# sdroh1027/DiffusionVID

Hardware: AMD Instinct MI355X
Metric: frames/sec (1000x600) DiffusionVID-R101 x1 (higher is better)
Workload: dtype f16

## Files before the change

diffusionvid_amd/csrc/bneck.hip:

```cpp
#include <stdlib.h>

#include "../../include/dvid_hip.h"
#include "common.h"
#include "igemm_epilogue.h"
#include "kernels.h"
#include "options.h"

namespace {

__device__ __attribute__((aligned(16))) unsigned int g_zero16_bn[4] = {0u, 0u, 0u, 0u};

typedef unsigned int uint4v __attribute__((ext_vector_type(4)));

template <int N>
__device__ __forceinline__ void bn_wait_vmcnt() {
    asm volatile("s_waitcnt vmcnt(%0)" ::"n"(N) : "memory");
}
__device__ __forceinline__ void bn_glds16(const void* gsrc, char* lds_wave_base) {
    __builtin_amdgcn_global_load_lds((const __attribute__((address_space(1))) void*)gsrc,
                                     (__attribute__((address_space(3))) void*)lds_wave_base, 16, 0, 0);
}
__device__ __forceinline__ float bn_mix_add_lo(unsigned int h2, float x) {
    float d;
    asm("v_fma_mix_f32 %0, %1, 1.0, %2 op_sel_hi:[1,0,0]" : "=v"(d) : "v"(h2), "v"(x));
    return d;
}
__device__ __forceinline__ float bn_mix_add_hi(unsigned int h2, float x) {
    float d;
    asm("v_fma_mix_f32 %0, %1, 1.0, %2 op_sel:[1,0,0] op_sel_hi:[1,0,0]" : "=v"(d) : "v"(h2), "v"(x));
    return d;
}

constexpr int TH = 8, TW = 32;
constexpr int HH = TH + 2, HW = 34;
constexpr int PXB = 128;
constexpr int A_PIECES = 48;
constexpr int kHalo = 0;
constexpr int kW2 = A_PIECES * 1024;
constexpr int kW3 = kW2 + 9 * 8192;
constexpr int kBias = kW3 + 32768;
constexpr int kBytes = 160 * 1024;

struct BneckParams {
    const half_t* t1;
    const half_t* w2;
    const float* b2;
    const half_t* w3;
    const float* b3;
    const half_t* res;
    const half_t* ws;
    const float* bs;
    const half_t* w1n;
    const float* b1n;
    half_t* out;
    half_t* t1n;
    int H, W, nrows, tiles_x, ntiles;
};

__device__ __forceinline__ void bn_swap(const float16v& acc, unsigned int (&u)[16]) {
#pragma unroll
    for (int r = 0; r < 16; ++r) {
        const float f = acc[r];
        u[r] = __float_as_uint(f);
    }
#pragma unroll
    for (int g = 0; g < 2; ++g)
#pragma unroll
        for (int r = 0; r < 4; ++r) {
            const auto sw = __builtin_amdgcn_permlane32_swap(u[8 * g + r], u[8 * g + 4 + r], false, false);
            u[8 * g + r] = sw[0];
            u[8 * g + 4 + r] = sw[1];
        }
}

template <bool SC, int TN>
__global__ __launch_bounds__(512) void bneck64_tail_kernel(BneckParams p) {
    constexpr bool TAIL = TN > 0;
    constexpr int NT1 = TN > 0 ? TN / 32 : 1;
    constexpr int kW1 = TN == 128 ? kW2 : kHalo;
    static_assert(TN == 0 || TN == 64 || (TN == 128 && !SC), "next conv1: 64 channels, or 128 without a shortcut in the same launch");
    extern __shared__ __attribute__((aligned(16))) char smem[];
    const int tid = threadIdx.x, lane = tid & 63;
    const int wave = __builtin_amdgcn_readfirstlane(tid >> 6);
    const int hi = lane >> 5, frow = lane & 31;
    const int lid = igemm_xcd_remap((int)blockIdx.x, p.ntiles);
    const int tx = lid % p.tiles_x, ty = lid / p.tiles_x;
    const int r0 = ty * TH, x0 = tx * TW;
    const char* zero = reinterpret_cast<const char*>(g_zero16_bn);

    if (wave < 4) {
        const float* src = wave == 0 ? p.b2 : wave == 1 ? p.b3 : wave == 2 ? (TAIL ? p.b1n : nullptr) : (SC ? p.bs : nullptr);
        const int n16 = (wave & 1) ? 64 : (wave == 2 ? TN / 4 : 16);
        bn_glds16(src && lane < n16 ? reinterpret_cast<const char*>(src + lane * 4) : zero, smem + kBias + wave * 1024);
    }
    const int prow = lane >> 3, pslot = lane & 7;
#pragma unroll
    for (int i = 0; i < A_PIECES / 8; ++i) {
        const int q = wave + 8 * i;
        const int pidx = 8 * q + prow;
        const int hy = pidx / HW, hx = pidx - hy * HW;
        const int gr = r0 - 1 + hy, gx = x0 - 1 + hx;
        const bool ok = pidx < HH * HW && (unsigned)gr < (unsigned)p.nrows && (unsigned)gx < (unsigned)p.W;
        const int lch = pslot ^ ((hx >> 1) & 7);
        bn_glds16(ok ? reinterpret_cast<const char*>(p.t1 + ((long)gr * p.W + gx) * 64 + lch * 8) : zero, smem + kHalo + q * 1024);
    }
    const int wrow = 8 * wave + prow;
    const int wlch = pslot ^ ((wrow >> 1) & 7);
    const char* const w2src = reinterpret_cast<const char*>(p.w2 + (long)wrow * 576 + wlch * 8);
#pragma unroll
    for (int tap = 0; tap < 3; ++tap) bn_glds16(w2src + tap * 128, smem + kW2 + tap * 8192 + wave * 1024);
    asm volatile("" ::: "memory");
#pragma unroll
    for (int tap = 3; tap < 9; ++tap) bn_glds16(w2src + tap * 128, smem + kW2 + tap * 8192 + wave * 1024);
#pragma unroll
    for (int i = 0; i < 4; ++i) {
        const int row = 64 * i + wrow;
        bn_glds16(reinterpret_cast<const char*>(p.w3 + (long)row * 64 + wlch * 8), smem + kW3 + i * 8192 + wave * 1024);
    }
    asm volatile("" ::: "memory");

    const int gr = r0 + wave, gx = x0 + frow;
    const bool valid = gr < p.nrows && gx < p.W;
    const long pix = (long)(gr < p.nrows ? gr : p.nrows - 1) * p.W + (gx < p.W ? gx : p.W - 1);
    constexpr int NRES = SC ? 4 : 16;
    half8 resv[NRES];
    int a_off[3][4];
#pragma unroll
    for (int dx = 0; dx < 3; ++dx)
#pragma unroll
        for (int ks = 0; ks < 4; ++ks) {
            const int hx = dx + frow;
            a_off[dx][ks] = hx * PXB + (((2 * ks + hi) ^ ((hx >> 1) & 7)) << 4);
        }
    int b_off[4];
#pragma unroll
    for (int ks = 0; ks < 4; ++ks) b_off[ks] = frow * PXB + (((2 * ks + hi) ^ ((frow >> 1) & 7)) << 4);
    const int yimg = (r0 + wave) % p.H;
    const bool up_ok = yimg > 0, down_ok = yimg < p.H - 1;

    float16v acc2[2];
#pragma unroll
    for (int j = 0; j < 2; ++j)
#pragma unroll
        for (int r = 0; r < 16; ++r) acc2[j][r] = 0.f;

    auto conv2_tap = [&](int tap) {
        const int dy = tap / 3, dx = tap % 3;
        if ((dy == 0 && !up_ok) || (dy == 2 && !down_ok)) return;
        const char* bst = smem + kW2 + tap * 8192;
        const char* hrow = smem + kHalo + (wave + dy) * (HW * PXB);
        half8 fw[2][4], fp[4];
#pragma unroll
        for (int ks = 0; ks < 4; ++ks) {
            fp[ks] = *reinterpret_cast<const half8*>(hrow + a_off[dx][ks]);
#pragma unroll
            for (int j = 0; j < 2; ++j) fw[j][ks] = *reinterpret_cast<const half8*>(bst + j * 4096 + b_off[ks]);
        }
#pragma unroll
        for (int ks = 0; ks < 4; ++ks)
#pragma unroll
            for (int j = 0; j < 2; ++j) acc2[j] = __builtin_amdgcn_mfma_f32_32x32x16_f16(fw[j][ks], fp[ks], acc2[j], 0, 0, 0);
    };

    bn_wait_vmcnt<10>();
    asm volatile("s_waitcnt lgkmcnt(0)" ::: "memory");
    __builtin_amdgcn_s_barrier();
#pragma unroll
    for (int tap = 0; tap < 3; ++tap) conv2_tap(tap);
    bn_wait_vmcnt<0>();
    __builtin_amdgcn_s_barrier();
    asm volatile("" ::: "memory");
    if (SC) {
#pragma unroll
        for (int ks = 0; ks < 4; ++ks) resv[ks] = *reinterpret_cast<const half8*>(p.res + pix * 64 + 16 * ks + 8 * hi);
    } else {
#pragma unroll
        for (int k = 0; k < 16; ++k) resv[k] = *reinterpret_cast<const half8*>(p.res + pix * 256 + 16 * k + 8 * hi);
    }
    asm volatile("" ::: "memory");
#pragma unroll
    for (int tap = 3; tap < 9; ++tap) conv2_tap(tap);
    asm volatile("s_waitcnt lgkmcnt(0)" ::: "memory");
    __builtin_amdgcn_s_barrier();
    asm volatile("" ::: "memory");

    if (TAIL) {
#pragma unroll
        for (int c = 0; c < 4; ++c)
#pragma unroll
            for (int i = 0; i < TN / 64; ++i)
                bn_glds16(reinterpret_cast<const char*>(p.w1n + (long)(64 * i + wrow) * 256 + c * 64 + wlch * 8),
                          smem + kW1 + c * (TN * 128) + (8 * i + wave) * 1024);
    }
    if (SC) {
#pragma unroll
        for (int i = 0; i < 4; ++i) {
            const int row = 64 * i + wrow;
            bn_glds16(reinterpret_cast<const char*>(p.ws + (long)row * 64 + wlch * 8), smem + kW2 + i * 8192 + wave * 1024);
        }
    }
    asm volatile("" ::: "memory");

    const float* const bl = reinterpret_cast<const float*>(smem + kBias);
    half8 t2f[4];
#pragma unroll
    for (int j = 0; j < 2; ++j) {
        unsigned int u[16];
        bn_swap(acc2[j], u);
#pragma unroll
        for (int g = 0; g < 2; ++g) {
            const float4v blo = *reinterpret_cast<const float4v*>(bl + 32 * j + 16 * g + 8 * hi);
            const float4v bhi = *reinterpret_cast<const float4v*>(bl + 32 * j + 16 * g + 8 * hi + 4);
            float4v lo, hv;
#pragma unroll
            for (int e = 0; e < 4; ++e) {
                lo[e] = __uint_as_float(u[8 * g + e]) + blo[e];
                hv[e] = __uint_as_float(u[8 * g + 4 + e]) + bhi[e];
            }
            const half4 hlo = __builtin_convertvector(lo, half4), hhi = __builtin_convertvector(hv, half4);
            half8 o = __builtin_shufflevector(hlo, hhi, 0, 1, 2, 3, 4, 5, 6, 7);
            t2f[2 * j + g] = __builtin_elementwise_max(o, half8{0, 0, 0, 0, 0, 0, 0, 0});
        }
    }
    if (TAIL || SC) {
        bn_wait_vmcnt<0>();
        __builtin_amdgcn_s_barrier();
        asm volatile("" ::: "memory");
    }

    half8 outf[16];
    half_t* const orow = p.out + ((long)gr * p.W + gx) * 256 + 8 * hi;
#pragma unroll
    for (int jj = 0; jj < 8; ++jj) {
        half8 fw3[4];
#pragma unroll
        for (int ks = 0; ks < 4; ++ks) fw3[ks] = *reinterpret_cast<const half8*>(smem + kW3 + jj * 4096 + b_off[ks]);
        float16v acc3;
#pragma unroll
        for (int r = 0; r < 16; ++r) acc3[r] = 0.f;
#pragma unroll
        for (int ks = 0; ks < 4; ++ks) acc3 = __builtin_amdgcn_mfma_f32_32x32x16_f16(fw3[ks], t2f[ks], acc3, 0, 0, 0);
        unsigned int us[16];
        if (SC) {
            half8 fws[4];
#pragma unroll
            for (int ks = 0; ks < 4; ++ks) fws[ks] = *reinterpret_cast<const half8*>(smem + kW2 + jj * 4096 + b_off[ks]);
            float16v accs;
#pragma unroll
            for (int r = 0; r < 16; ++r) accs[r] = 0.f;
#pragma unroll
            for (int ks = 0; ks < 4; ++ks) accs = __builtin_amdgcn_mfma_f32_32x32x16_f16(fws[ks], resv[ks], accs, 0, 0, 0);
            bn_swap(accs, us);
        }
        unsigned int u[16];
        bn_swap(acc3, u);
#pragma unroll
        for (int g = 0; g < 2; ++g) {
            const int c0 = 32 * jj + 16 * g + 8 * hi;
            const float4v blo = *reinterpret_cast<const float4v*>(bl + 256 + c0);
            const float4v bhi = *reinterpret_cast<const float4v*>(bl + 256 + c0 + 4);
            float4v lo, hv;
#pragma unroll
            for (int e = 0; e < 4; ++e) {
                lo[e] = __uint_as_float(u[8 * g + e]) + blo[e];
                hv[e] = __uint_as_float(u[8 * g + 4 + e]) + bhi[e];
            }
            uint4v rr;
            if (SC) {
                const float4v slo = *reinterpret_cast<const float4v*>(bl + 768 + c0);
                const float4v shi = *reinterpret_cast<const float4v*>(bl + 768 + c0 + 4);
                float4v a, b;
#pragma unroll
                for (int e = 0; e < 4; ++e) {
                    a[e] = __uint_as_float(us[8 * g + e]) + slo[e];
                    b[e] = __uint_as_float(us[8 * g + 4 + e]) + shi[e];
                }
                const half4 ha = __builtin_convertvector(a, half4), hb = __builtin_convertvector(b, half4);
                rr = __builtin_bit_cast(uint4v, __builtin_shufflevector(ha, hb, 0, 1, 2, 3, 4, 5, 6, 7));
            } else {
                rr = __builtin_bit_cast(uint4v, resv[2 * jj + g]);
            }
            lo[0] = bn_mix_add_lo(rr[0], lo[0]);
            lo[1] = bn_mix_add_hi(rr[0], lo[1]);
            lo[2] = bn_mix_add_lo(rr[1], lo[2]);
            lo[3] = bn_mix_add_hi(rr[1], lo[3]);
            hv[0] = bn_mix_add_lo(rr[2], hv[0]);
            hv[1] = bn_mix_add_hi(rr[2], hv[1]);
            hv[2] = bn_mix_add_lo(rr[3], hv[2]);
            hv[3] = bn_mix_add_hi(rr[3], hv[3]);
            const half4 hlo = __builtin_convertvector(lo, half4), hhi = __builtin_convertvector(hv, half4);
            half8 o = __builtin_shufflevector(hlo, hhi, 0, 1, 2, 3, 4, 5, 6, 7);
            o = __builtin_elementwise_max(o, half8{0, 0, 0, 0, 0, 0, 0, 0});
            outf[2 * jj + g] = o;
            if (valid) *reinterpret_cast<half8*>(orow + 32 * jj + 16 * g) = o;
        }
    }

    if (TAIL) {
        float16v acc1[NT1];
#pragma unroll
        for (int j = 0; j < NT1; ++j)
#pragma unroll
            for (int r = 0; r < 16; ++r) acc1[j][r] = 0.f;
#pragma unroll
        for (int k = 0; k < 16; ++k) {
            const char* wt = smem + kW1 + (k >> 2) * (TN * 128) + b_off[k & 3];
#pragma unroll
            for (int j = 0; j < NT1; ++j) {
                const half8 fw = *reinterpret_cast<const half8*>(wt + j * 4096);
                acc1[j] = __builtin_amdgcn_mfma_f32_32x32x16_f16(fw, outf[k], acc1[j], 0, 0, 0);
            }
        }
        half_t* const trow = p.t1n + ((long)gr * p.W + gx) * TN + 8 * hi;
#pragma unroll
        for (int j = 0; j < NT1; ++j) {
            unsigned int u[16];
            bn_swap(acc1[j], u);
#pragma unroll
            for (int g = 0; g < 2; ++g) {
                const float4v blo = *reinterpret_cast<const float4v*>(bl + 512 + 32 * j + 16 * g + 8 * hi);
                const float4v bhi = *reinterpret_cast<const float4v*>(bl + 512 + 32 * j + 16 * g + 8 * hi + 4);
                float4v lo, hv;
#pragma unroll
                for (int e = 0; e < 4; ++e) {
                    lo[e] = __uint_as_float(u[8 * g + e]) + blo[e];
                    hv[e] = __uint_as_float(u[8 * g + 4 + e]) + bhi[e];
                }
                const half4 hlo = __builtin_convertvector(lo, half4), hhi = __builtin_convertvector(hv, half4);
                half8 o = __builtin_shufflevector(hlo, hhi, 0, 1, 2, 3, 4, 5, 6, 7);
                o = __builtin_elementwise_max(o, half8{0, 0, 0, 0, 0, 0, 0, 0});
                if (valid) *reinterpret_cast<half8*>(trow + 32 * j + 16 * g) = o;
            }
        }
    }
}

template <bool SC, int TN>
int bn_launch(const BneckParams& p, hipStream_t s) {
    static_assert(kBytes <= 160 * 1024, "LDS");
    static std::atomic<unsigned long long> attr_set{0};
    if (first_on_device(attr_set)) {
        HIP_TRY(hipFuncSetAttribute(reinterpret_cast<const void*>(&bneck64_tail_kernel<SC, TN>), hipFuncAttributeMaxDynamicSharedMemorySize, kBytes));
        mark_on_device(attr_set);
    }
    const int lds_opt = g_opt.bneck_lds;
    hipLaunchKernelGGL((bneck64_tail_kernel<SC, TN>), dim3(p.ntiles), dim3(512), lds_opt >= kBias + 4096 && lds_opt <= kBytes ? lds_opt : kBytes, s, p);
    LAUNCH_CHECK();
    return DVID_OK;
}


constexpr int H8_PIECES = 88;
constexpr int k8Ring = H8_PIECES * 1024;
constexpr int k8Stage = 16384;
constexpr int k8Bias = k8Ring + 4 * k8Stage;
constexpr int k8Bytes = 160 * 1024;

struct Bneck128Params {
    const half_t* t1;
    const half_t* w2;
    const float* b2;
    const half_t* w3;
    const float* b3;
    const half_t* res;
    const half_t* w1n;
    const float* b1n;
    half_t* out;
    half_t* t1n;
    int H, W, nrows, tiles_x, ntiles;
};

__device__ __forceinline__ void bn_wait_vmcnt_n(int n) {
    switch (n) {
        case 0: bn_wait_vmcnt<0>(); break;
        case 1: bn_wait_vmcnt<1>(); break;
        case 2: bn_wait_vmcnt<2>(); break;
        case 3: bn_wait_vmcnt<3>(); break;
        case 4: bn_wait_vmcnt<4>(); break;
        case 5: bn_wait_vmcnt<5>(); break;
        case 6: bn_wait_vmcnt<6>(); break;
        case 7: bn_wait_vmcnt<7>(); break;
        case 8: bn_wait_vmcnt<8>(); break;
        case 9: bn_wait_vmcnt<9>(); break;
        default: bn_wait_vmcnt<10>(); break;
    }
}

template <bool CONV2, bool TAIL>
__global__ __launch_bounds__(512) void bneck128_tail_kernel(Bneck128Params p) {
    constexpr int NC2 = CONV2 ? 18 : 0, NST = NC2 + 16, D3 = TAIL ? 2 : 1;
    extern __shared__ __attribute__((aligned(16))) char smem[];
    const int tid = threadIdx.x, lane = tid & 63;
    const int wave = __builtin_amdgcn_readfirstlane(tid >> 6);
    const int hi = lane >> 5, frow = lane & 31;
    const int lid = igemm_xcd_remap((int)blockIdx.x, p.ntiles);
    const int tx = lid % p.tiles_x, ty = lid / p.tiles_x;
    const int r0 = ty * TH, x0 = tx * TW;
    const char* zero = reinterpret_cast<const char*>(g_zero16_bn);
    char* const ring = smem + k8Ring;

    auto dma_cnt = [](int t) { return (t < 0 || t >= NST) ? 0 : (t < NC2 ? 2 : D3); };
    auto r_cnt = [&](int u) { return (u >= NC2 && u < NC2 + 12) ? 2 : 0; };
    auto wait_n = [&](int s) { return dma_cnt(s + 1) + dma_cnt(s + 2) + r_cnt(s - 3) + r_cnt(s - 2) + r_cnt(s - 1); };

    if (wave < 3) {
        const float* src = wave < 2 ? p.b3 + wave * 256 + lane * 4 : (lane < 32 ? p.b2 + lane * 4 : (TAIL ? p.b1n + (lane - 32) * 4 : nullptr));
        bn_glds16(src ? reinterpret_cast<const char*>(src) : zero, smem + k8Bias + wave * 1024);
    }
    const int gr = r0 + wave, gx = x0 + frow;
    const bool valid = gr < p.nrows && gx < p.W;
    const long pix = (long)(gr < p.nrows ? gr : p.nrows - 1) * p.W + (gx < p.W ? gx : p.W - 1);
    const half_t* const rrow = p.res + pix * 512 + 8 * hi;
    half8 resr[4][2];
    half8 t2f[8];
    char* const rring = smem + wave * (5 * 2048);
    auto issue_res = [&](int jn) {
#pragma unroll
        for (int g = 0; g < 2; ++g) bn_glds16(reinterpret_cast<const char*>(rrow + 32 * jn + 16 * g), rring + (jn % 5) * 2048 + g * 1024);
    };
#pragma unroll
    for (int jj = 0; jj < 4; ++jj)
#pragma unroll
        for (int g = 0; g < 2; ++g) resr[jj][g] = *reinterpret_cast<const half8*>(rrow + 32 * jj + 16 * g);
    asm volatile("" ::: "memory");
    if (CONV2) {
#pragma unroll
        for (int i = 0; i < H8_PIECES / 8; ++i) {
            const int q = wave + 8 * i;
            const int pidx = 4 * q + (lane >> 4);
            const int hy = pidx / HW, hx = pidx - hy * HW;
            const int hgr = r0 - 1 + hy, hgx = x0 - 1 + hx;
            const bool ok = pidx < HH * HW && (unsigned)hgr < (unsigned)p.nrows && (unsigned)hgx < (unsigned)p.W;
            const int lch = (lane & 15) ^ (hx & 15);
            bn_glds16(ok ? reinterpret_cast<const char*>(p.t1 + ((long)hgr * p.W + hgx) * 128 + lch * 8) : zero, smem + q * 1024);
        }
    } else {
#pragma unroll
        for (int k = 0; k < 8; ++k) t2f[k] = *reinterpret_cast<const half8*>(p.t1 + pix * 128 + 16 * k + 8 * hi);
    }
    asm volatile("" ::: "memory");

    const int prow = lane >> 3, pslot = lane & 7;
    const int wrow = 8 * wave + prow;
    const char* const w2src = CONV2 ? reinterpret_cast<const char*>(p.w2 + (long)wrow * 1152 + (pslot ^ ((wrow >> 1) & 7)) * 8) : zero;
    const int q3 = wave & 3, kh3 = wave >> 2, row3 = 8 * q3 + prow;
    const char* const w3src = reinterpret_cast<const char*>(p.w3 + (long)row3 * 128 + kh3 * 64 + (pslot ^ ((row3 >> 1) & 7)) * 8);
    const int rown = 16 * wave + (lane >> 2);
    const char* const w1src = TAIL ? reinterpret_cast<const char*>(p.w1n + (long)rown * 512 + ((lane & 3) ^ ((rown >> 2) & 3)) * 8) : zero;
    auto issue_step = [&](int t) {
        if (t >= NST) return;
        char* const stg = ring + (t & 3) * k8Stage;
        if (t < NC2) {
            const int koff = ((t >> 1) * 128 + (t & 1) * 64) * 2;
            bn_glds16(w2src + koff, stg + wave * 1024);
            bn_glds16(w2src + koff + 64 * 1152 * 2, stg + (wave + 8) * 1024);
        } else {
            const int jj = t - NC2;
            bn_glds16(w3src + (long)jj * (32 * 128 * 2), stg + kh3 * 4096 + q3 * 1024);
            if (TAIL) bn_glds16(w1src + jj * 64, stg + 8192 + wave * 1024);
        }
    };
    issue_step(0);
    issue_step(1);
    issue_step(2);
    asm volatile("" ::: "memory");

    int b_off[4];
#pragma unroll
    for (int ks = 0; ks < 4; ++ks) b_off[ks] = frow * PXB + (((2 * ks + hi) ^ ((frow >> 1) & 7)) << 4);
    const float* const bl = reinterpret_cast<const float*>(smem + k8Bias);

    if (CONV2) {
        const int yimg = (r0 + wave) % p.H;
        const bool up_ok = yimg > 0, down_ok = yimg < p.H - 1;
        int a_base[3], a_key[3];
#pragma unroll
        for (int dx = 0; dx < 3; ++dx) {
            a_base[dx] = (dx + frow) * 256;
            a_key[dx] = (dx + frow) & 15;
        }
        float16v acc2[4];
#pragma unroll
        for (int j = 0; j < 4; ++j)
#pragma unroll
            for (int r = 0; r < 16; ++r) acc2[j][r] = 0.f;
#pragma unroll
        for (int s = 0; s < NC2; ++s) {
            bn_wait_vmcnt_n(wait_n(s));
            __builtin_amdgcn_s_barrier();
            asm volatile("" ::: "memory");
            issue_step(s + 3);
            const int tap = s >> 1, kh = s & 1, dy = tap / 3, dx = tap % 3;
            if (!((dy == 0 && !up_ok) || (dy == 2 && !down_ok))) {
                const char* stg = ring + (s & 3) * k8Stage;
                const char* hrow = smem + (wave + dy) * (HW * 256) + a_base[dx];
                half8 fp[4];
#pragma unroll
                for (int ks = 0; ks < 4; ++ks) fp[ks] = *reinterpret_cast<const half8*>(hrow + (((2 * (4 * kh + ks) + hi) ^ a_key[dx]) << 4));
#pragma unroll
                for (int ks = 0; ks < 4; ++ks) {
                    half8 fw[4];
#pragma unroll
                    for (int j = 0; j < 4; ++j) fw[j] = *reinterpret_cast<const half8*>(stg + j * 4096 + b_off[ks]);
#pragma unroll
                    for (int j = 0; j < 4; ++j) acc2[j] = __builtin_amdgcn_mfma_f32_32x32x16_f16(fw[j], fp[ks], acc2[j], 0, 0, 0);
                }
            }
            asm volatile("" ::: "memory");
        }
#pragma unroll
        for (int j = 0; j < 4; ++j) {
            unsigned int u[16];
            bn_swap(acc2[j], u);
#pragma unroll
            for (int g = 0; g < 2; ++g) {
                const float4v blo = *reinterpret_cast<const float4v*>(bl + 512 + 32 * j + 16 * g + 8 * hi);
                const float4v bhi = *reinterpret_cast<const float4v*>(bl + 512 + 32 * j + 16 * g + 8 * hi + 4);
                float4v lo, hv;
#pragma unroll
                for (int e = 0; e < 4; ++e) {
                    lo[e] = __uint_as_float(u[8 * g + e]) + blo[e];
                    hv[e] = __uint_as_float(u[8 * g + 4 + e]) + bhi[e];
                }
                const half4 hlo = __builtin_convertvector(lo, half4), hhi = __builtin_convertvector(hv, half4);
                half8 o = __builtin_shufflevector(hlo, hhi, 0, 1, 2, 3, 4, 5, 6, 7);
                t2f[2 * j + g] = __builtin_elementwise_max(o, half8{0, 0, 0, 0, 0, 0, 0, 0});
            }
        }
    }

    float16v acc1[4];
#pragma unroll
    for (int j = 0; j < 4; ++j)
#pragma unroll
        for (int r = 0; r < 16; ++r) acc1[j][r] = 0.f;
    half_t* const orow = p.out + ((long)gr * p.W + gx) * 512 + 8 * hi;
#pragma unroll
    for (int jj = 0; jj < 16; ++jj) {
        const int s = NC2 + jj;
        bn_wait_vmcnt_n(wait_n(s));
        __builtin_amdgcn_s_barrier();
        asm volatile("" ::: "memory");
        issue_step(s + 3);
        if (jj < 12) issue_res(jj + 4);
        asm volatile("" ::: "memory");
        const char* stg = ring + (s & 3) * k8Stage;
        float16v acc3;
#pragma unroll
        for (int r = 0; r < 16; ++r) acc3[r] = 0.f;
#pragma unroll
        for (int kk = 0; kk < 8; ++kk) {
            const half8 fw = *reinterpret_cast<const half8*>(stg + (kk >> 2) * 4096 + b_off[kk & 3]);
            acc3 = __builtin_amdgcn_mfma_f32_32x32x16_f16(fw, t2f[kk], acc3, 0, 0, 0);
        }
        unsigned int u[16];
        bn_swap(acc3, u);
        half8 outf[2];
#pragma unroll
        for (int g = 0; g < 2; ++g) {
            const int c0 = 32 * jj + 16 * g + 8 * hi;
            const float4v blo = *reinterpret_cast<const float4v*>(bl + c0);
            const float4v bhi = *reinterpret_cast<const float4v*>(bl + c0 + 4);
            float4v lo, hv;
#pragma unroll
            for (int e = 0; e < 4; ++e) {
                lo[e] = __uint_as_float(u[8 * g + e]) + blo[e];
                hv[e] = __uint_as_float(u[8 * g + 4 + e]) + bhi[e];
            }
            const uint4v rr = jj < 4 ? __builtin_bit_cast(uint4v, resr[jj & 3][g])
                                     : *reinterpret_cast<const uint4v*>(rring + (jj % 5) * 2048 + g * 1024 + lane * 16);
            lo[0] = bn_mix_add_lo(rr[0], lo[0]);
            lo[1] = bn_mix_add_hi(rr[0], lo[1]);
            lo[2] = bn_mix_add_lo(rr[1], lo[2]);
            lo[3] = bn_mix_add_hi(rr[1], lo[3]);
            hv[0] = bn_mix_add_lo(rr[2], hv[0]);
            hv[1] = bn_mix_add_hi(rr[2], hv[1]);
            hv[2] = bn_mix_add_lo(rr[3], hv[2]);
            hv[3] = bn_mix_add_hi(rr[3], hv[3]);
            const half4 hlo = __builtin_convertvector(lo, half4), hhi = __builtin_convertvector(hv, half4);
            half8 o = __builtin_shufflevector(hlo, hhi, 0, 1, 2, 3, 4, 5, 6, 7);
            o = __builtin_elementwise_max(o, half8{0, 0, 0, 0, 0, 0, 0, 0});
            outf[g] = o;
            if (valid) *reinterpret_cast<half8*>(orow + 32 * jj + 16 * g) = o;
        }
        if (TAIL) {
#pragma unroll
            for (int g = 0; g < 2; ++g)
#pragma unroll
                for (int j = 0; j < 4; ++j) {
                    const half8 fw = *reinterpret_cast<const half8*>(stg + 8192 + j * 2048 + frow * 64 + (((2 * g + hi) ^ ((frow >> 2) & 3)) << 4));
                    acc1[j] = __builtin_amdgcn_mfma_f32_32x32x16_f16(fw, outf[g], acc1[j], 0, 0, 0);
                }
        }
        asm volatile("" ::: "memory");
    }

    if (TAIL) {
        half_t* const trow = p.t1n + ((long)gr * p.W + gx) * 128 + 8 * hi;
#pragma unroll
        for (int j = 0; j < 4; ++j) {
            unsigned int u[16];
            bn_swap(acc1[j], u);
#pragma unroll
            for (int g = 0; g < 2; ++g) {
                const float4v blo = *reinterpret_cast<const float4v*>(bl + 640 + 32 * j + 16 * g + 8 * hi);
                const float4v bhi = *reinterpret_cast<const float4v*>(bl + 640 + 32 * j + 16 * g + 8 * hi + 4);
                float4v lo, hv;
#pragma unroll
                for (int e = 0; e < 4; ++e) {
                    lo[e] = __uint_as_float(u[8 * g + e]) + blo[e];
                    hv[e] = __uint_as_float(u[8 * g + 4 + e]) + bhi[e];
                }
                const half4 hlo = __builtin_convertvector(lo, half4), hhi = __builtin_convertvector(hv, half4);
                half8 o = __builtin_shufflevector(hlo, hhi, 0, 1, 2, 3, 4, 5, 6, 7);
                o = __builtin_elementwise_max(o, half8{0, 0, 0, 0, 0, 0, 0, 0});
                if (valid) *reinterpret_cast<half8*>(trow + 32 * j + 16 * g) = o;
            }
        }
    }
}

template <bool CONV2, bool TAIL>
int bn128_launch(const Bneck128Params& p, hipStream_t s) {
    static_assert(k8Bytes <= 160 * 1024, "LDS");
    static std::atomic<unsigned long long> attr_set{0};
    if (first_on_device(attr_set)) {
        HIP_TRY(hipFuncSetAttribute(reinterpret_cast<const void*>(&bneck128_tail_kernel<CONV2, TAIL>), hipFuncAttributeMaxDynamicSharedMemorySize, k8Bytes));
        mark_on_device(attr_set);
    }
    const int lds_opt = g_opt.bneck_lds;
    hipLaunchKernelGGL((bneck128_tail_kernel<CONV2, TAIL>), dim3(p.ntiles), dim3(512), lds_opt >= k8Bias + 3072 && lds_opt <= k8Bytes ? lds_opt : k8Bytes, s, p);
    LAUNCH_CHECK();
    return DVID_OK;
}

}

int dvid_igemm_set_bottleneck_fusion(int mode) {
    if (mode < -1 || mode > 2) return DVID_ERR_ARG;
    g_opt.bneck_fuse = mode < 0 ? DvidOptions().bneck_fuse : mode;
    return DVID_OK;
}
bool dvid_bneck64_tail_preferred(int H, int W) {
    const int mode = g_opt.bneck_fuse;
    if (!mode) return false;
    if (mode >= 2) return true;
    return ceil_div(W, TW) * TW * 7 <= W * 8 && H * W >= 512;
}

int dvid_bneck64_tail_launch(const half_t* t1, const half_t* w2, const float* b2, const half_t* w3, const float* b3, const half_t* res,
                             const half_t* ws, const float* bs, const half_t* w1n, const float* b1n, int n_next, half_t* out, half_t* t1n,
                             int n, int H, int W, hipStream_t s) {
    if (!t1 || !w2 || !b2 || !w3 || !b3 || !res || !out || n <= 0 || H <= 0 || W <= 0) return DVID_ERR_ARG;
    if ((ws && !bs) || (w1n && (!b1n || !t1n))) return DVID_ERR_ARG;
    if (w1n && n_next != 64 && !(n_next == 128 && !ws)) return DVID_ERR_UNSUPPORTED;
    BneckParams p;
    p.t1 = t1;
    p.w2 = w2;
    p.b2 = b2;
    p.w3 = w3;
    p.b3 = b3;
    p.res = res;
    p.ws = ws;
    p.bs = bs;
    p.w1n = w1n;
    p.b1n = b1n;
    p.out = out;
    p.t1n = t1n;
    p.H = H;
    p.W = W;
    p.nrows = n * H;
    p.tiles_x = ceil_div(W, TW);
    p.ntiles = p.tiles_x * ceil_div(p.nrows, TH);
    if (ws) return w1n ? bn_launch<true, 64>(p, s) : bn_launch<true, 0>(p, s);
    if (!w1n) return bn_launch<false, 0>(p, s);
    return n_next == 128 ? bn_launch<false, 128>(p, s) : bn_launch<false, 64>(p, s);
}

int dvid_bneck128_tail_launch(const half_t* t1, const half_t* w2, const float* b2, const half_t* w3, const float* b3, const half_t* res,
                              const half_t* w1n, const float* b1n, half_t* out, half_t* t1n, int n, int H, int W, hipStream_t s) {
    if (!t1 || !w3 || !b3 || !res || !out || n <= 0 || H <= 0 || W <= 0) return DVID_ERR_ARG;
    if ((w2 && !b2) || (w1n && (!b1n || !t1n))) return DVID_ERR_ARG;
    Bneck128Params p;
    p.t1 = t1;
    p.w2 = w2;
    p.b2 = b2 ? b2 : b3;
    p.w3 = w3;
    p.b3 = b3;
    p.res = res;
    p.w1n = w1n;
    p.b1n = b1n;
    p.out = out;
    p.t1n = t1n;
    p.H = H;
    p.W = W;
    p.nrows = n * H;
    p.tiles_x = ceil_div(W, TW);
    p.ntiles = p.tiles_x * ceil_div(p.nrows, TH);
    if (w2) return w1n ? bn128_launch<true, true>(p, s) : bn128_launch<true, false>(p, s);
    return w1n ? bn128_launch<false, true>(p, s) : bn128_launch<false, false>(p, s);
}
```

diffusionvid_amd/csrc/model.hip:

```cpp
#include <math.h>
#include <stdarg.h>
#include <stdlib.h>
#include <string.h>

#include <map>
#include <mutex>
#include <string>
#include <vector>

#include "../../include/dvid_hip.h"
#include "common.h"
#include "kernels.h"
#include "options.h"

DvidOptions g_opt;

namespace {

thread_local char g_err[512] = "";
void set_err(const char* fmt, ...) {
    va_list ap;
    va_start(ap, fmt);
    vsnprintf(g_err, sizeof(g_err), fmt, ap);
    va_end(ap);
// ... 1088 lines not shown
}

int dvid_model_destroy(dvid_model* m) {
    if (!m) return DVID_OK;
    for (void* p : m->owned) (void)hipFree(p);
    DevBuf* bufs[] = {&m->img8, &m->bufX, &m->bufY, &m->bufT1, &m->bufT2, &m->bufSC, &m->c3, &m->c4, &m->c5, &m->lat[0], &m->sw_x, &m->sw_x2, &m->sw_ln16, &m->sw_qkv16, &m->sw_attn16, &m->sw_h16,
                      &m->lat[1], &m->lat[2], &m->roi, &m->params, &m->dyn, &m->qkv, &m->attn16, &m->f32a, &m->f32b, &m->f32c,
                      &m->f32d, &m->h16a, &m->h16b, &m->hid16, &m->ss, &m->deltas, &m->kvproj, &m->mem16, &m->splitk, &m->vt};
    for (DevBuf* b : bufs) b->release();
    for (DevBuf& b : m->ss_slabs) b.release();
    delete m;
    return DVID_OK;
}

int dvid_model_set_tensor(dvid_model* m, const char* name, const float* data, const int64_t* shape, int ndim) {
    g_err[0] = 0;
    if (!m || !name || !data || ndim < 0 || ndim > 8) FAIL(DVID_ERR_ARG, "bad argument");
    if (m->finalized) FAIL(DVID_ERR_STATE, "model already finalized");
    HostTensor t;
    t.shape.assign(shape, shape + ndim);
    t.v.assign(data, data + t.numel());
    m->raw[name] = std::move(t);
    return DVID_OK;
}

int dvid_model_finalize(dvid_model* m) {
    g_err[0] = 0;
    if (!m) FAIL(DVID_ERR_ARG, "null model");
    if (m->finalized) return DVID_OK;
    const dvid_config& c = m->cfg;
    m->has_backbone = c.backbone_type == 1 ? c.swin_depths[0] > 0 : c.res_blocks[0] > 0;
    if (m->has_backbone && c.backbone_type == 0) {
        const std::string bu = "backbone.bottom_up.";
        TRY(make_conv_bn(m, bu + "stem.conv1", 2, 3, 8, &m->stem));
        TRY(make_stem_s2d(m, bu + "stem.conv1", &m->stem_s2d));
        for (int s = 0; s < 4; ++s) {
            m->blocks[s].resize(c.res_blocks[s]);
            for (int b = 0; b < c.res_blocks[s]; ++b) {
                const std::string p = bu + "res" + std::to_string(s + 2) + "." + std::to_string(b);
                Block& blk = m->blocks[s][b];
                const int stride = (b == 0 && s > 0) ? 2 : 1;
                TRY(make_conv_bn(m, p + ".conv1", 1, 0, 0, &blk.c1));
                TRY(make_conv_bn(m, p + ".conv2", stride, 1, 0, &blk.c2));
                TRY(make_conv_bn(m, p + ".conv3", 1, 0, 0, &blk.c3));
                blk.has_sc = (b == 0);
                if (blk.has_sc) TRY(make_conv_bn(m, p + ".shortcut", stride, 0, 0, &blk.sc));
            }
        }
    }
    if (m->has_backbone && c.backbone_type == 1) {
        if (c.swin_window != 7) FAIL(DVID_ERR_UNSUPPORTED, "Swin window size %d (only 7 is built)", c.swin_window);
        const std::string bu = "backbone.bottom_up.";
        {
            NEED(pw, bu + "patch_embed.proj.weight");
            NEED(pb, bu + "patch_embed.proj.bias");
            if (pw->shape[2] != 4 || pw->shape[3] != 4) FAIL(DVID_ERR_UNSUPPORTED, "patch size must be 4");
            TRY(make_conv(m, *pw, {}, pb->v, 4, 0, 8, nullptr, &m->swin_patch));
            TRY(make_ln(m, bu + "patch_embed.norm", &m->swin_patch_norm));
        }
        int relidx[49][49];
        for (int i = 0; i < 49; ++i)
            for (int j = 0; j < 49; ++j) relidx[i][j] = ((i / 7 - j / 7) + 6) * 13 + ((i % 7 - j % 7) + 6);
        for (int st = 0; st < 4; ++st) {
            SwinStageW& S = m->swin[st];
            S.dim = c.swin_embed_dim << st;
            S.heads = c.swin_heads[st];
            if (S.dim != S.heads * 32) FAIL(DVID_ERR_UNSUPPORTED, "Swin stage %d: head dim %d != 32", st, S.dim / S.heads);
            S.blocks.resize(c.swin_depths[st]);
            for (int b = 0; b < c.swin_depths[st]; ++b) {
                const std::string p = bu + "layers." + std::to_string(st) + ".blocks." + std::to_string(b);
                SwinBlockW& B = S.blocks[b];
                TRY(make_ln(m, p + ".norm1", &B.norm1));
                TRY(make_ln(m, p + ".norm2", &B.norm2));
                TRY(make_linear(m, p + ".attn.qkv", true, &B.qkv));
                TRY(make_linear(m, p + ".attn.proj", true, &B.proj));
                TRY(make_linear(m, p + ".mlp.fc1", true, &B.fc1));
                TRY(make_linear(m, p + ".mlp.fc2", true, &B.fc2));
                NEED(qb, p + ".attn.qkv.bias");
                std::vector<half_t> qb16(qb->v.size());
                for (size_t i = 0; i < qb16.size(); ++i) qb16[i] = f2h(qb->v[i]);
                TRY(m->upload(qb16.data(), qb16.size() * sizeof(half_t), reinterpret_cast<void**>(&B.qkv_bias16)));
                NEED(tb, p + ".attn.relative_position_bias_table");
                if (tb->shape[0] != 169 || tb->shape[1] != S.heads) FAIL(DVID_ERR_ARG, "%s: bad bias table shape", p.c_str());
                std::vector<float> rb((size_t)S.heads * 49 * SWIN_RELBIAS_PITCH, 0.f);
                for (int h = 0; h < S.heads; ++h)
                    for (int i = 0; i < 49; ++i)
                        for (int j = 0; j < 49; ++j)
                            rb[((size_t)h * 49 + i) * SWIN_RELBIAS_PITCH + j] = tb->v[(size_t)relidx[i][j] * S.heads + h];
                TRY(upload_f32(m, rb, &B.relbias));
            }
            S.has_down = st < 3;
            if (S.has_down) {
                const std::string p = bu + "layers." + std::to_string(st) + ".downsample";
                TRY(make_ln(m, p + ".norm", &S.down_norm));
                TRY(make_linear(m, p + ".reduction", false, &S.down_red));
            }
            S.has_out = st >= 1;
            if (S.has_out) TRY(make_ln(m, bu + "norm" + std::to_string(st), &S.out_norm));
        }
    }
    if (m->has_backbone) {
        for (int l = 0; l < 3; ++l) {
            const std::string lat = "backbone.fpn_lateral" + std::to_string(l + 3);
            const std::string outn = "backbone.fpn_output" + std::to_string(l + 3);
            NEED(lw, lat + ".weight");
            NEED(lb, lat + ".bias");
            NEED(ow, outn + ".weight");
            NEED(ob, outn + ".bias");
            TRY(make_conv(m, *lw, {}, lb->v, 1, 0, 0, nullptr, &m->lateral[l]));
            TRY(make_conv(m, *ow, {}, ob->v, 1, 1, 0, nullptr, &m->output[l]));
        }
    }
    m->heads.resize(c.num_heads);
    for (int i = 0; i < c.num_heads; ++i) TRY(make_head(m, "head.head_series." + std::to_string(i), false, &m->heads[i]));
    m->heads_cond.resize(c.num_heads_cond);
    for (int i = 0; i < c.num_heads_cond; ++i)
        TRY(make_head(m, "head.head_series_cond." + std::to_string(i), true, &m->heads_cond[i]));
    if (m->get("head.global_attention.0.0.in_proj_weight")) {
        const int d = c.hidden_dim;
        TRY(make_linear(m, "head.global_attention.0.0.in_proj", true, &m->gq, nullptr, 0, d));
        TRY(make_linear(m, "head.global_attention.0.0.in_proj", true, &m->gkv, nullptr, d, 2 * d));
        TRY(make_linear(m, "head.global_attention.0.0.out_proj", true, &m->gout));
    }
    {
        NEED(w1, "head.time_mlp.1.weight");
        NEED(b1, "head.time_mlp.1.bias");
        NEED(w3, "head.time_mlp.3.weight");
        NEED(b3, "head.time_mlp.3.bias");
        m->tm1_w = w1->v;
        m->tm1_b = b1->v;
        m->tm3_w = w3->v;
        m->tm3_b = b3->v;
    }
    m->raw.clear();
    m->finalized = true;
    return DVID_OK;
}

int dvid_model_set_precision(dvid_model* m, int precision) {
    g_err[0] = 0;
    if (!m || (precision != 0 && precision != 1)) FAIL(DVID_ERR_ARG, "precision must be 0 (float16) or 1 (float32)");
    if (m->finalized) FAIL(DVID_ERR_STATE, "dvid_model_set_precision must precede dvid_model_finalize (the weights are packed for one precision)");
    m->precision = precision;
    return DVID_OK;
}

namespace {
struct OptEntry {
    const char* name;
    int DvidOptions::*field;
    int lo, hi;
};
const OptEntry kOptions[] = {
    {"conv3x3", &DvidOptions::conv3x3, 0, 2},       {"wstat", &DvidOptions::wstat, 0, 2},           {"bneck_fuse", &DvidOptions::bneck_fuse, 0, 2},
    {"stem_pool", &DvidOptions::stem_pool, 0, 1},   {"head_tail", &DvidOptions::head_tail, 0, 1},   {"roi_fuse", &DvidOptions::roi_fuse, 0, 1},   {"ln_rows", &DvidOptions::ln_rows, 0, 1},
    {"igemm_cfg", &DvidOptions::igemm_cfg, -1, 255}, {"igemm_tune", &DvidOptions::igemm_tune, -1, 1}, {"igemm_generic", &DvidOptions::igemm_generic, 0, 1},
    {"f32_split", &DvidOptions::f32_split, 0, 1},    {"f32_wstat", &DvidOptions::f32_wstat, 0, 2},    {"f32_conv3x3", &DvidOptions::f32_conv3x3, 0, 1},
    {"bneck_lds", &DvidOptions::bneck_lds, 0, 160 * 1024},
};
}

int dvid_set_option(const char* name, int value) {
    g_err[0] = 0;
    if (!name) FAIL(DVID_ERR_ARG, "null option name");
    for (const OptEntry& e : kOptions)
        if (!strcmp(e.name, name)) {
            if (value < e.lo || value > e.hi) FAIL(DVID_ERR_ARG, "option %s: %d outside [%d, %d]", name, value, e.lo, e.hi);
            if (e.field == &DvidOptions::igemm_cfg && value >= dvid_igemm_num_configs()) FAIL(DVID_ERR_ARG, "igemm_cfg %d: the table has %d entries", value, dvid_igemm_num_configs());
            g_opt.*(e.field) = value;
            return DVID_OK;
        }
    FAIL(DVID_ERR_ARG, "unknown option '%s'", name);
}

int dvid_get_option(const char* name, int* value) {
    g_err[0] = 0;
    if (!name || !value) FAIL(DVID_ERR_ARG, "null argument");
    for (const OptEntry& e : kOptions)
        if (!strcmp(e.name, name)) {
            *value = g_opt.*(e.field);
            return DVID_OK;
        }
    FAIL(DVID_ERR_ARG, "unknown option '%s'", name);
}

int dvid_reset_options(void) {
    g_opt = DvidOptions();
    return DVID_OK;
}

int dvid_effective_config(char* buf, int cap) {
    g_err[0] = 0;
    if (!buf || cap <= 0) FAIL(DVID_ERR_ARG, "no buffer");
    std::string out;
    for (const OptEntry& e : kOptions) out += std::string(e.name) + "=" + std::to_string(g_opt.*(e.field)) + " ";
    for (const char* env : {"DVID_IGEMM_TUNE", "DVID_IGEMM_TUNE_CACHE", "DVID_CHAINS", "DVID_POISON_WORKSPACE"}) {
        const char* v = getenv(env);
        out += std::string(env) + "=" + (v ? v : "") + " ";
    }
    if (!out.empty()) out.pop_back();
    if ((int)out.size() + 1 > cap) FAIL(DVID_ERR_ARG, "buffer of %d bytes, need %d", cap, (int)out.size() + 1);
    memcpy(buf, out.c_str(), out.size() + 1);
    return DVID_OK;
}

int dvid_model_take_range_flag(dvid_model* m, int* exceeded, void* stream) {
    g_err[0] = 0;
    if (!m || !exceeded) FAIL(DVID_ERR_ARG, "null argument");
    *exceeded = 0;
    if (!m->f32_range_flag) return DVID_OK;
    hipStream_t s = reinterpret_cast<hipStream_t>(stream);
    HIP_TRY(hipMemcpyAsync(exceeded, m->f32_range_flag, sizeof(int), hipMemcpyDeviceToHost, s));
    HIP_TRY(hipStreamSynchronize(s));
    if (*exceeded) HIP_TRY(hipMemsetAsync(m->f32_range_flag, 0, sizeof(int), s));
    return DVID_OK;
}

int dvid_set_stem_pool(int mode) {
    if (mode < -1 || mode > 1) return DVID_ERR_ARG;
    g_opt.stem_pool = mode < 0 ? DvidOptions().stem_pool : mode;
    return DVID_OK;
}

unsigned long long dvid_workspace_generation(const dvid_model* m) { return m ? m->ws_gen.load(std::memory_order_relaxed) : 0ull; }

int dvid_set_chains(dvid_model* m, int nchain) {
    g_err[0] = 0;
    if (!m || nchain < 1 || nchain > 4) FAIL(DVID_ERR_ARG, "nchain must be 1..4");
    m->nchain = nchain;
    return DVID_OK;
}

int dvid_set_stem_layout(dvid_model* m, int space_to_depth) {
    g_err[0] = 0;
    if (!m) FAIL(DVID_ERR_ARG, "null model");
    m->use_s2d = space_to_depth != 0;
    return DVID_OK;
}

int dvid_workspace_reserve(dvid_model* m, int max_frames, int height, int width, int boxes_per_frame) {
    g_err[0] = 0;
    if (!m || max_frames <= 0 || boxes_per_frame <= 0) FAIL(DVID_ERR_ARG, "bad argument");
    if (height % 32 || width % 32) FAIL(DVID_ERR_ARG, "height/width must be multiples of 32 (got %dx%d)", height, width);
    const size_t n = ((size_t)max_frames + 3) / 4 * 4;
    const size_t px4 = (size_t)(height / 4) * (width / 4);
    const size_t es = m->precision == 1 ? 2 : 1;
    if (m->has_backbone && m->cfg.backbone_type == 1) {
        const size_t C0 = m->cfg.swin_embed_dim, M0 = n * px4;
        TRY(m->img8.ensure(n * height * width * 8 * 2, &m->ws_gen));
        TRY(m->sw_x.ensure(M0 * C0 * 4, &m->ws_gen));
        TRY(m->sw_x2.ensure(M0 * C0 * 4 / 2, &m->ws_gen));
        TRY(m->sw_ln16.ensure(M0 * C0 * 2 * es, &m->ws_gen));
        TRY(m->sw_qkv16.ensure(M0 * C0 * 3 * 2 * es, &m->ws_gen));
        TRY(m->sw_attn16.ensure(M0 * C0 * 2 * es, &m->ws_gen));
        TRY(m->sw_h16.ensure(M0 * C0 * 4 * 2 * es, &m->ws_gen));
        TRY(m->c3.ensure(n * (px4 / 4) * (C0 * 2) * 2 * es, &m->ws_gen));
        TRY(m->c4.ensure(n * (px4 / 16) * (C0 * 4) * 2 * es, &m->ws_gen));
        TRY(m->c5.ensure(n * (px4 / 64) * (C0 * 8) * 2 * es, &m->ws_gen));
        for (int l = 0; l < 3; ++l) TRY(m->lat[l].ensure(n * (px4 / (4 << (2 * l))) * 256 * 2 * es, &m->ws_gen));
    }
    if (m->has_backbone && m->cfg.backbone_type == 0) {
        TRY(m->img8.ensure(n * height * width * 8 * 2, &m->ws_gen));
        const size_t big = n * px4 * 256 * 2 * es;
        TRY(m->bufX.ensure(big, &m->ws_gen));
        TRY(m->bufY.ensure(big, &m->ws_gen));
        TRY(m->bufT1.ensure(big, &m->ws_gen));
        TRY(m->bufT2.ensure(big, &m->ws_gen));
        TRY(m->bufSC.ensure(big, &m->ws_gen));
        TRY(m->c3.ensure(n * (px4 / 4) * 512 * 2 * es, &m->ws_gen));
        TRY(m->c4.ensure(n * (px4 / 16) * 1024 * 2 * es, &m->ws_gen));
        TRY(m->c5.ensure(n * (px4 / 64) * 2048 * 2 * es, &m->ws_gen));
        for (int l = 0; l < 3; ++l) TRY(m->lat[l].ensure(n * (px4 / (4 << (2 * l))) * 256 * 2 * es, &m->ws_gen));
    }
    const size_t R = n * boxes_per_frame;
    const int d = m->cfg.hidden_dim;
    TRY(m->roi.ensure(R * 49 * d * 2 * es, &m->ws_gen));
    TRY(m->dyn.ensure(R * 49 * d * 2 * es, &m->ws_gen));
    TRY(m->params.ensure(R * 2 * d * m->cfg.dim_dynamic * 2 * es, &m->ws_gen));
    TRY(m->qkv.ensure(R * 3 * d * 4, &m->ws_gen));
    TRY(m->attn16.ensure(R * d * 2 * es, &m->ws_gen));
    TRY(m->f32a.ensure(R * d * 4, &m->ws_gen));
    TRY(m->f32b.ensure(R * d * 4, &m->ws_gen));
    TRY(m->f32c.ensure(R * d * 4, &m->ws_gen));
    TRY(m->f32d.ensure(R * d * 4, &m->ws_gen));
    TRY(m->h16a.ensure(R * d * 2 * es, &m->ws_gen));
    TRY(m->h16b.ensure(R * d * 2 * es, &m->ws_gen));
    TRY(m->hid16.ensure(R * m->cfg.dim_feedforward * 2 * es, &m->ws_gen));
    TRY(m->ss.ensure((size_t)(m->cfg.num_heads + m->cfg.num_heads_cond) * n * 2 * d * 4, &m->ws_gen));
    TRY(m->deltas.ensure(R * 4 * 4, &m->ws_gen));
    TRY(m->splitk.ensure(R * d * 4 * 8, &m->ws_gen));
    TRY(m->vt.ensure((size_t)n * m->cfg.nheads * 32 * (((size_t)boxes_per_frame + 31) / 32 * 32 + 32) * 2, &m->ws_gen));
    m->ws_frames = max_frames;
    m->ws_h = height;
    m->ws_w = width;
    m->ws_boxes = boxes_per_frame;
    return DVID_OK;
}

int dvid_backbone_resnet_fpn(dvid_model* m, const float* images, int n, int height, int width, void* p3, void* p4, void* p5,
                             void* stream) {
    if (!images || n <= 0) {
        g_err[0] = 0;
        FAIL(DVID_ERR_ARG, "no images");
    }
    std::vector<const float*> frames(n);
    for (int i = 0; i < n; ++i) frames[i] = images + (size_t)i * 3 * height * width;
    return dvid_backbone_resnet_fpn_frames(m, frames.data(), n, height, width, p3, p4, p5, stream);
// ... 640 lines not shown
```

Before: 2386.

## Make bottleneck tail kernel persistent with next-tile halo prefetch and resident conv2 weights

Converts the fused ResNet bottleneck 64-channel tail kernel into a persistent kernel. Each workgroup loops over about four tiles, keeps most conv2 tap weights resident in LDS, and prefetches the next tile's halo while the conv3, shortcut and next-conv1 epilogue runs. The aim is to cut repeated weight loads and per-tile launch and fill latency. In exchange, the weight region is time-shared with the shortcut and next-conv1 weights, so some taps must be reloaded each iteration. The grid also shrinks, which may reduce parallelism on small feature maps.

New measurement: 2385, median of 6. About the same (-0.0%).

```diff
diff --git a/diffusionvid_amd/csrc/bneck.hip b/diffusionvid_amd/csrc/bneck.hip
--- a/diffusionvid_amd/csrc/bneck.hip
+++ b/diffusionvid_amd/csrc/bneck.hip
@@ -73,19 +73,22 @@
         }
 }
 
-template <bool SC, int TN>
+template <bool SC, int TN, bool PERS>
 __global__ __launch_bounds__(512) void bneck64_tail_kernel(BneckParams p) {
     constexpr bool TAIL = TN > 0;
     constexpr int NT1 = TN > 0 ? TN / 32 : 1;
-    constexpr int kW1 = TN == 128 ? kW2 : kHalo;
+    constexpr int OV = (SC ? 32768 : 0) + TN * 512;
+    constexpr int kWS = PERS ? kW2 + 9 * 8192 - OV : kW2;
+    constexpr int kW1 = PERS ? kWS + (SC ? 32768 : 0) : (TN == 128 ? kW2 : kHalo);
+    constexpr int TAP_KEEP = 9 - OV / 8192;
     static_assert(TN == 0 || TN == 64 || (TN == 128 && !SC), "next conv1: 64 channels, or 128 without a shortcut in the same launch");
+    static_assert(OV % 8192 == 0 && TAP_KEEP >= 1, "the time-shared weights end the tap region");
     extern __shared__ __attribute__((aligned(16))) char smem[];
     const int tid = threadIdx.x, lane = tid & 63;
     const int wave = __builtin_amdgcn_readfirstlane(tid >> 6);
     const int hi = lane >> 5, frow = lane & 31;
-    const int lid = igemm_xcd_remap((int)blockIdx.x, p.ntiles);
-    const int tx = lid % p.tiles_x, ty = lid / p.tiles_x;
-    const int r0 = ty * TH, x0 = tx * TW;
+    int vb = blockIdx.x;
+    int lid = igemm_xcd_remap(vb, p.ntiles);
     const char* zero = reinterpret_cast<const char*>(g_zero16_bn);
 
     if (wave < 4) {
@@ -94,16 +97,20 @@
         bn_glds16(src && lane < n16 ? reinterpret_cast<const char*>(src + lane * 4) : zero, smem + kBias + wave * 1024);
     }
     const int prow = lane >> 3, pslot = lane & 7;
-#pragma unroll
-    for (int i = 0; i < A_PIECES / 8; ++i) {
-        const int q = wave + 8 * i;
-        const int pidx = 8 * q + prow;
-        const int hy = pidx / HW, hx = pidx - hy * HW;
-        const int gr = r0 - 1 + hy, gx = x0 - 1 + hx;
-        const bool ok = pidx < HH * HW && (unsigned)gr < (unsigned)p.nrows && (unsigned)gx < (unsigned)p.W;
-        const int lch = pslot ^ ((hx >> 1) & 7);
-        bn_glds16(ok ? reinterpret_cast<const char*>(p.t1 + ((long)gr * p.W + gx) * 64 + lch * 8) : zero, smem + kHalo + q * 1024);
-    }
+    auto issue_halo = [&](int plid, bool live) {
+        const int hr0 = (plid / p.tiles_x) * TH, hx0 = (plid % p.tiles_x) * TW;
+#pragma unroll
+        for (int i = 0; i < A_PIECES / 8; ++i) {
+            const int q = wave + 8 * i;
+            const int pidx = 8 * q + prow;
+            const int hy = pidx / HW, hx = pidx - hy * HW;
+            const int gr = hr0 - 1 + hy, gx = hx0 - 1 + hx;
+            const bool ok = live && pidx < HH * HW && (unsigned)gr < (unsigned)p.nrows && (unsigned)gx < (unsigned)p.W;
+            const int lch = pslot ^ ((hx >> 1) & 7);
+            bn_glds16(ok ? reinterpret_cast<const char*>(p.t1 + ((long)gr * p.W + gx) * 64 + lch * 8) : zero, smem + kHalo + q * 1024);
+        }
+    };
+    issue_halo(lid, true);
     const int wrow = 8 * wave + prow;
     const int wlch = pslot ^ ((wrow >> 1) & 7);
     const char* const w2src = reinterpret_cast<const char*>(p.w2 + (long)wrow * 576 + wlch * 8);
@@ -119,6 +126,11 @@
     }
     asm volatile("" ::: "memory");
 
+    for (;;) {
+    const int tx = lid % p.tiles_x, ty = lid / p.tiles_x;
+    const int r0 = ty * TH, x0 = tx * TW;
+    const int vnext = vb + (int)gridDim.x;
+    const bool has_next = PERS && vnext < p.ntiles;
     const int gr = r0 + wave, gx = x0 + frow;
     const bool valid = gr < p.nrows && gx < p.W;
     const long pix = (long)(gr < p.nrows ? gr : p.nrows - 1) * p.W + (gx < p.W ? gx : p.W - 1);
@@ -162,14 +174,21 @@
             for (int j = 0; j < 2; ++j) acc2[j] = __builtin_amdgcn_mfma_f32_32x32x16_f16(fw[j][ks], fp[ks], acc2[j], 0, 0, 0);
     };
 
-    bn_wait_vmcnt<10>();
-    asm volatile("s_waitcnt lgkmcnt(0)" ::: "memory");
-    __builtin_amdgcn_s_barrier();
-#pragma unroll
-    for (int tap = 0; tap < 3; ++tap) conv2_tap(tap);
-    bn_wait_vmcnt<0>();
-    __builtin_amdgcn_s_barrier();
-    asm volatile("" ::: "memory");
+    if (PERS) {
+        bn_wait_vmcnt<0>();
+        asm volatile("s_waitcnt lgkmcnt(0)" ::: "memory");
+        __builtin_amdgcn_s_barrier();
+        asm volatile("" ::: "memory");
+    } else {
+        bn_wait_vmcnt<10>();
+        asm volatile("s_waitcnt lgkmcnt(0)" ::: "memory");
+        __builtin_amdgcn_s_barrier();
+#pragma unroll
+        for (int tap = 0; tap < 3; ++tap) conv2_tap(tap);
+        bn_wait_vmcnt<0>();
+        __builtin_amdgcn_s_barrier();
+        asm volatile("" ::: "memory");
+    }
     if (SC) {
 #pragma unroll
         for (int ks = 0; ks < 4; ++ks) resv[ks] = *reinterpret_cast<const half8*>(p.res + pix * 64 + 16 * ks + 8 * hi);
@@ -179,10 +198,14 @@
     }
     asm volatile("" ::: "memory");
 #pragma unroll
-    for (int tap = 3; tap < 9; ++tap) conv2_tap(tap);
+    for (int tap = PERS ? 0 : 3; tap < 9; ++tap) conv2_tap(tap);
     asm volatile("s_waitcnt lgkmcnt(0)" ::: "memory");
     __builtin_amdgcn_s_barrier();
     asm volatile("" ::: "memory");
+    if (PERS) {
+#pragma unroll
+        for (int k = 0; k < NRES; ++k) asm volatile("" ::"v"(resv[k]));
+    }
 
     if (TAIL) {
 #pragma unroll
@@ -196,9 +219,10 @@
 #pragma unroll
         for (int i = 0; i < 4; ++i) {
             const int row = 64 * i + wrow;
-            bn_glds16(reinterpret_cast<const char*>(p.ws + (long)row * 64 + wlch * 8), smem + kW2 + i * 8192 + wave * 1024);
-        }
-    }
+            bn_glds16(reinterpret_cast<const char*>(p.ws + (long)row * 64 + wlch * 8), smem + kWS + i * 8192 + wave * 1024);
+        }
+    }
+    if (PERS) issue_halo(igemm_xcd_remap(has_next ? vnext : vb, p.ntiles), has_next);
     asm volatile("" ::: "memory");
 
     const float* const bl = reinterpret_cast<const float*>(smem + kBias);
@@ -223,7 +247,10 @@
         }
     }
     if (TAIL || SC) {
-        bn_wait_vmcnt<0>();
+        if (PERS)
+            bn_wait_vmcnt<A_PIECES / 8>();
+        else
+            bn_wait_vmcnt<0>();
         __builtin_amdgcn_s_barrier();
         asm volatile("" ::: "memory");
     }
@@ -244,7 +271,7 @@
         if (SC) {
             half8 fws[4];
 #pragma unroll
-            for (int ks = 0; ks < 4; ++ks) fws[ks] = *reinterpret_cast<const half8*>(smem + kW2 + jj * 4096 + b_off[ks]);
+            for (int ks = 0; ks < 4; ++ks) fws[ks] = *reinterpret_cast<const half8*>(smem + kWS + jj * 4096 + b_off[ks]);
             float16v accs;
 #pragma unroll
             for (int r = 0; r < 16; ++r) accs[r] = 0.f;
@@ -333,20 +360,45 @@
             }
         }
     }
-}
-
-template <bool SC, int TN>
+
+    if (!has_next) break;
+    vb = vnext;
+    lid = igemm_xcd_remap(vb, p.ntiles);
+    if (OV > 0) {
+        asm volatile("s_waitcnt lgkmcnt(0)" ::: "memory");
+        __builtin_amdgcn_s_barrier();
+        asm volatile("" ::: "memory");
+#pragma unroll
+        for (int tap = TAP_KEEP; tap < 9; ++tap) bn_glds16(w2src + tap * 128, smem + kW2 + tap * 8192 + wave * 1024);
+        asm volatile("" ::: "memory");
+    }
+    }
+}
+
+constexpr int kPatchesPerWg = 4;
+int bn_persistent_grid(int ntiles) {
+    const int g = (ceil_div(ntiles, kPatchesPerWg) + 7) & ~7;
+    return ntiles < g ? ntiles : g;
+}
+
+template <bool SC, int TN, bool PERS>
 int bn_launch(const BneckParams& p, hipStream_t s) {
     static_assert(kBytes <= 160 * 1024, "LDS");
     static std::atomic<unsigned long long> attr_set{0};
     if (first_on_device(attr_set)) {
-        HIP_TRY(hipFuncSetAttribute(reinterpret_cast<const void*>(&bneck64_tail_kernel<SC, TN>), hipFuncAttributeMaxDynamicSharedMemorySize, kBytes));
+        HIP_TRY(hipFuncSetAttribute(reinterpret_cast<const void*>(&bneck64_tail_kernel<SC, TN, PERS>), hipFuncAttributeMaxDynamicSharedMemorySize, kBytes));
         mark_on_device(attr_set);
     }
     const int lds_opt = g_opt.bneck_lds;
-    hipLaunchKernelGGL((bneck64_tail_kernel<SC, TN>), dim3(p.ntiles), dim3(512), lds_opt >= kBias + 4096 && lds_opt <= kBytes ? lds_opt : kBytes, s, p);
+    const int grid = PERS ? bn_persistent_grid(p.ntiles) : p.ntiles;
+    hipLaunchKernelGGL((bneck64_tail_kernel<SC, TN, PERS>), dim3(grid), dim3(512), lds_opt >= kBias + 4096 && lds_opt <= kBytes ? lds_opt : kBytes, s, p);
     LAUNCH_CHECK();
     return DVID_OK;
+}
+
+template <bool SC, int TN>
+int bn_launch(const BneckParams& p, hipStream_t s) {
+    return g_opt.bneck_fuse == 3 ? bn_launch<SC, TN, false>(p, s) : bn_launch<SC, TN, true>(p, s);
 }
 
 
@@ -637,14 +689,14 @@
 }
 
 int dvid_igemm_set_bottleneck_fusion(int mode) {
-    if (mode < -1 || mode > 2) return DVID_ERR_ARG;
+    if (mode < -1 || mode > 3) return DVID_ERR_ARG;
     g_opt.bneck_fuse = mode < 0 ? DvidOptions().bneck_fuse : mode;
     return DVID_OK;
 }
 bool dvid_bneck64_tail_preferred(int H, int W) {
     const int mode = g_opt.bneck_fuse;
     if (!mode) return false;
-    if (mode >= 2) return true;
+    if (mode == 2) return true;
     return ceil_div(W, TW) * TW * 7 <= W * 8 && H * W >= 512;
 }
 
diff --git a/diffusionvid_amd/csrc/model.hip b/diffusionvid_amd/csrc/model.hip
--- a/diffusionvid_amd/csrc/model.hip
+++ b/diffusionvid_amd/csrc/model.hip
@@ -1264,7 +1264,7 @@
     int lo, hi;
 };
 const OptEntry kOptions[] = {
-    {"conv3x3", &DvidOptions::conv3x3, 0, 2},       {"wstat", &DvidOptions::wstat, 0, 2},           {"bneck_fuse", &DvidOptions::bneck_fuse, 0, 2},
+    {"conv3x3", &DvidOptions::conv3x3, 0, 2},       {"wstat", &DvidOptions::wstat, 0, 2},           {"bneck_fuse", &DvidOptions::bneck_fuse, 0, 3},
     {"stem_pool", &DvidOptions::stem_pool, 0, 1},   {"head_tail", &DvidOptions::head_tail, 0, 1},   {"roi_fuse", &DvidOptions::roi_fuse, 0, 1},   {"ln_rows", &DvidOptions::ln_rows, 0, 1},
     {"igemm_cfg", &DvidOptions::igemm_cfg, -1, 255}, {"igemm_tune", &DvidOptions::igemm_tune, -1, 1}, {"igemm_generic", &DvidOptions::igemm_generic, 0, 1},
     {"f32_split", &DvidOptions::f32_split, 0, 1},    {"f32_wstat", &DvidOptions::f32_wstat, 0, 2},    {"f32_conv3x3", &DvidOptions::f32_conv3x3, 0, 1},
```
